# ai4ce/DiscoNet

Measured on AMD Instinct MI355X. Metric: scenes/sec (5-agent 256x256 BEV), higher is better.
Workload: dtype f16 hi+lo pair per value (32 bits; 22-bit significand for |x| >= 0.125, f16 exponent range, lo subnormal below: absolute floor 2^-25); conv products as split-f16 x3 MFMA, f32 accumulate; 1 GPU; DiscoNet det eval forward (--com disco), 5-agent, batch 4 per GPU, 256x256x13 BEV, no KD, sparse voxel lists -> dense -> enc -> DiscoGraph fusion -> dec -> cls/reg heads; agents=5, batch_per_gpu=4, conv_math=sp, launch=hipGraph replay, parallelism=scene-parallel x1 (no data-path collective)

## Files before the change

### disconet_amd/_lib.py

```python
import ctypes
import os
from ctypes import (POINTER, Structure, c_char_p, c_double, c_float, c_int, c_int32, c_long, c_longlong, c_size_t,
                    c_uint64, c_void_p)

_HERE = os.path.dirname(os.path.abspath(__file__))
LIB_PATH = os.environ.get("DISCONET_HIP_LIB") or os.path.join(_HERE, "libdisconet_hip.so")


class DnError(RuntimeError):
    pass


class ConvDesc(Structure):
    _fields_ = [(n, c_int32) for n in (
        "n_images", "h_in", "w_in", "c0", "c1", "up0", "c_out", "ksize", "stride", "relu",
        "ld0", "ld1", "ldo", "math")]


class PackJob(Structure):
    _fields_ = [("desc", ConvDesc), ("weight", c_void_p), ("packed", c_void_p), ("mode", c_int32), ("cin_total", c_int32),
                ("ci_first", c_int32), ("n_in", c_int32), ("wmul", c_float), ("reserved", c_int32)]


class FoldJob(Structure):
# ... 69 lines not shown
    "dn_conv_pack_multi_prepare": (c_int, [POINTER(PackJob), c_int, c_void_p, POINTER(c_int)]),
    "dn_conv_pack_weights_multi": (c_int, [c_void_p, c_int, c_int, c_void_p]),
    "dn_spconv2d": (c_int, [POINTER(ConvDesc), c_void_p, c_void_p, c_void_p, c_void_p, c_void_p,
                            c_void_p, c_void_p]),
    "dn_spconv_ks_supported": (c_int, [POINTER(ConvDesc), c_int]),
    "dn_spconv_workspace_bytes": (c_size_t, [POINTER(ConvDesc), c_int]),
    "dn_spconv2d_ks": (c_int, [POINTER(ConvDesc), c_int, c_void_p, c_void_p, c_void_p, c_void_p, c_void_p, c_void_p,
                               c_void_p, c_int, c_void_p, c_size_t, c_void_p]),
    "dn_spconv2d_pre_pair_supported": (c_int, [POINTER(ConvDesc), POINTER(ConvDesc)]),
    "dn_spconv2d_pre_pair": (c_int, [POINTER(ConvDesc), POINTER(ConvDesc), c_void_p, c_void_p, c_void_p, c_void_p, c_void_p,
                                     c_void_p, c_void_p, c_void_p, c_void_p]),
    "dn_spconv2d_dual": (c_int, [POINTER(ConvDesc), c_void_p, c_void_p, c_void_p, c_void_p, c_void_p,
                                 c_void_p, c_void_p, c_int, c_void_p]),
    "dn_spconv2d_nhwc": (c_int, [POINTER(ConvDesc), c_void_p, c_void_p, c_void_p, c_void_p, c_void_p, c_void_p, c_int,
                                 c_void_p]),
    "dn_sp_post1x1_packed_bytes": (c_size_t, []),
    "dn_sp_post1x1_pack_weights": (c_int, [c_void_p, c_int, c_int, c_float, c_void_p, c_void_p]),
    "dn_sp_post1x1_pack_heads": (c_int, [c_void_p, c_int, c_int, c_float, c_void_p, c_void_p]),
    "dn_spconv2d_post1x1": (c_int, [POINTER(ConvDesc), POINTER(Post1x1Desc)] + [c_void_p] * 8 +
                            [c_int, c_void_p, c_void_p, c_void_p]),
    "dn_spconv_force_config": (c_int, [c_int]),
    "dn_spconv_set_upmode": (c_int, [c_int]),
    "dn_spconv_last_form": (c_int, [POINTER(c_int), c_int]),
    "dn_conv_force_config": (c_int, [c_int]),
    "dn_conv_last_form": (c_int, [POINTER(c_int), c_int]),
    "dn_decode_boxes": (c_int, [c_void_p, c_void_p, c_void_p, c_int, c_long, c_void_p, c_void_p,
                                c_void_p]),
    "dn_detect_workspace_bytes": (c_size_t, [c_int, c_long, c_int]),
    "dn_detect": (c_int, [c_void_p, c_void_p, c_void_p, c_int, c_long, c_int, c_int, c_float, c_double, c_void_p,
                          c_void_p, c_void_p, c_void_p, c_void_p, c_size_t, c_void_p]),
    "dn_late_fuse_workspace_bytes": (c_size_t, [c_int, c_int, c_int, c_int, c_int, c_int]),
    "dn_late_fuse": (c_int, [c_void_p, c_void_p, c_void_p, c_void_p, c_void_p, c_int, c_int, c_int, c_int, c_int, c_int,
                             c_int, c_double, c_int, POINTER(c_double), c_void_p, c_void_p, c_void_p, c_void_p, c_void_p,
                             c_size_t, c_void_p]),
    "dn_ap_match_workspace_bytes": (c_size_t, [c_int, c_int, c_int, c_int]),
    "dn_ap_match": (c_int, [c_void_p, c_void_p, c_void_p, c_void_p, c_void_p, c_int, c_int, c_int, POINTER(c_double), c_int,
                            c_void_p, c_void_p, c_void_p, c_void_p, c_void_p, c_size_t, c_void_p, c_longlong, c_void_p, c_int,
                            c_int, c_void_p]),
    "dn_ap_reset": (c_int, [c_void_p, c_int, c_void_p]),
    "dn_gt_strata": (c_int, [c_void_p, c_void_p, c_void_p, c_int, c_int, c_int, POINTER(c_double), c_int, c_void_p, c_void_p]),
    "dn_ap_match_strata_workspace_bytes": (c_size_t, [c_int, c_int, c_int, c_int, c_int]),
    "dn_ap_match_strata": (c_int, [c_void_p, c_void_p, c_void_p, c_void_p, c_void_p, c_void_p, c_int, c_int, c_int,
                                   POINTER(c_double), c_int, c_int, c_void_p, c_void_p, c_void_p, c_void_p, c_void_p,
                                   c_void_p, c_size_t, c_void_p, c_longlong, c_void_p, c_int, c_int, c_void_p]),
    "dn_ap_strata_reset": (c_int, [c_void_p, c_int, c_int, c_void_p]),
    "dn_assign_targets_workspace_bytes": (c_size_t, [c_int, c_long, c_int]),
# ... 169 lines not shown
```

### disconet_amd/csrc/conv_sp.hip

```cpp
#ifndef DN_PHASE_TIMING
#define DN_PHASE_TIMING 0
#endif
#ifndef DN_SP_ABL
#define DN_SP_ABL 0
#endif
#include "dn_internal.h"
#include "sp_layout.h"
#include "sp_device.h"
#include "sp_split.h"
#include <array>
#include <cstdlib>
#include <type_traits>
#include <utility>

#if DN_PHASE_TIMING
__device__ unsigned long long g_phase_cycles[8];
extern "C" int dn_sp_phase_cycles(unsigned long long* host8, int reset) {
  if (hipDeviceSynchronize() != hipSuccess) return -1;
  if (host8 && hipMemcpyFromSymbol(host8, HIP_SYMBOL(g_phase_cycles), sizeof(unsigned long long) * 8) != hipSuccess) return -1;
  if (reset) { unsigned long long z[8] = {0}; if (hipMemcpyToSymbol(HIP_SYMBOL(g_phase_cycles), z, sizeof z) != hipSuccess) return -1; }
  return 0;
}
#endif

// ... 1146 lines not shown
             "spconv: a bit-grid source 0 (math = 4) needs a 3x3 stride-1 single-source layer of <= 32 channels");
  DN_REQUIRE(!d->up0 || (d->h_in % 2 == 0 && d->w_in % 2 == 0), "spconv: x2-upsampled source needs even h_in/w_in");
  DN_REQUIRE(d->c1 == 0 || (d->c0 % 16 == 0 && d->ksize == 3), "spconv: concat needs 3x3 and c0 %% 16 == 0 (c0 = %d)", d->c0);
  const size_t hs0 = d->up0 ? d->h_in / 2 : d->h_in, ws0 = d->up0 ? d->w_in / 2 : d->w_in;
  DN_REQUIRE(hs0 * ws0 * chunks_of(d->c0) * 64 < (1ull << 31) &&
                 (size_t)d->h_in * d->w_in * chunks_of(d->c1) * 64 < (1ull << 31),
             "spconv: one image must stay below 2 GiB");
  return DN_OK;
}

inline size_t packed_blocks(const dn_conv_desc& d) {
  const int nch = packed_chunks(d);
  if (up_mode(d) == 2) return dn::spq_packed_blocks(chunks_of(d.c0), nch);
  if (up_merged(d)) return (size_t)chunks_of(d.c0) * 12 + (size_t)(nch - chunks_of(d.c0)) * 9;
  return (size_t)nch * d.ksize * d.ksize;
}

enum SpCfgId { S3_256x64, S3_256x32, S3_128x64, S3_64x64, S3S2_128x64, S3S2_64x64, S1_256x64, S1_64x64,
               S3_256x64_T9, S3_512x64, S3_256x128, S1_256x64_C1, S3_256x32_ST, S3_64x64_T9, S3_128x64_T9,
               S3S2_64x64_T9, S3S2_128x64_T9, SP_CFG_COUNT };
enum SpForceId {
  FORCE_SPQ_BN32 = 20, FORCE_SPQ_BN64 = 21, FORCE_SPQ_DEEP = 22,
  FORCE_SPQ_ABL = 22,
  FORCE_TOOLS = 100,
  FORCE_ABL_256x64 = 100, FORCE_ABL_256x32 = 200,
  FORCE_ABL_64x64_T9 = 300,
  FORCE_ABL_S2_64x64 = 400,
};

template <int KS_, int STRIDE_, int TH_, int TW_, int BN_, int TG_, int CA_, int WAVES_M_, int WAVES_N_, int WTM_, int WTN_>
struct Geom {
  using G = Geom;
  static constexpr int KS = KS_, STRIDE = STRIDE_, TH = TH_, TW = TW_, BN = BN_, TG = TG_, CA = CA_, WAVES_M = WAVES_M_,
                       WAVES_N = WAVES_N_, WTM = WTM_, WTN = WTN_;
};
template <SpCfgId ID> struct Tile;
#define SP_TILE(id, bias_, deep_, ...) \
  template <> struct Tile<id> : __VA_ARGS__ { static constexpr float bias = bias_; static constexpr SpCfgId deep = deep_; }
SP_TILE(S3_256x64,      1.00f, S3_256x64_T9,   Geom<3, 1, 8,  32, 64,  3, 1, 4, 1, 2, 2>);
SP_TILE(S3_256x32,      1.15f, S3_256x32,      Geom<3, 1, 8,  32, 32,  3, 1, 4, 1, 2, 1>);
SP_TILE(S3_128x64,      1.10f, S3_128x64_T9,   Geom<3, 1, 8,  16, 64,  3, 1, 2, 2, 2, 1>);
SP_TILE(S3_64x64,       1.40f, S3_64x64_T9,    Geom<3, 1, 8,  8,  64,  3, 1, 2, 2, 1, 1>);
SP_TILE(S3S2_128x64,    1.45f, S3S2_128x64_T9, Geom<3, 2, 8,  16, 64,  3, 1, 2, 2, 2, 1>);
SP_TILE(S3S2_64x64,     1.00f, S3S2_64x64_T9,  Geom<3, 2, 8,  8,  64,  3, 1, 2, 2, 1, 1>);
SP_TILE(S1_256x64,      1.00f, S1_256x64,      Geom<1, 1, 8,  32, 64,  1, 2, 4, 1, 2, 2>);
SP_TILE(S1_64x64,       1.30f, S1_64x64,       Geom<1, 1, 8,  8,  64,  1, 4, 2, 2, 1, 1>);
// ... 356 lines not shown
}

extern "C" int dn_spconv_force_config(int cfg) {
  g_sp_force = cfg;
  return DN_OK;
}

extern "C" int dn_spconv_set_upmode(int mode) {
  g_sp_upmode = mode;
  return DN_OK;
}

namespace dn { SpLastForm g_sp_last_form = {-1, 0, 0, 0, 0, 0, 0, 0, 0, 0, 0, 0, 0, 0, 0, 0, 0, 0, 0, 0}; }

extern "C" int dn_spconv_last_form(int* out, int n) {
  constexpr int kInts = (int)(sizeof(dn::SpLastForm) / sizeof(int));
  static_assert(sizeof(dn::SpLastForm) == 20 * sizeof(int), "dn_spconv_last_form: the record is 20 ints");
  DN_REQUIRE(out && n > 0, "spconv last form: null pointer / no room");
  const int* f = reinterpret_cast<const int*>(&dn::g_sp_last_form);
  for (int i = 0; i < n && i < kInts; ++i) out[i] = f[i];
  return kInts;
}

namespace {
int spconv2d_impl(const dn_conv_desc* d, const void* src0, const void* src1, const void* packed, const float* scale,
                  const float* shift, void* out, float* out_nhwc, int ld_nhwc, void* stream, int kslices = 1,
                  void* workspace = nullptr, size_t workspace_bytes = 0);
}

extern "C" int dn_spconv2d(const dn_conv_desc* d, const void* src0, const void* src1,
                           const void* packed, const float* scale, const float* shift, void* out,
                           void* stream) {
  return spconv2d_impl(d, src0, src1, packed, scale, shift, out, nullptr, 0, stream);
}

extern "C" int dn_spconv2d_dual(const dn_conv_desc* d, const void* src0, const void* src1, const void* packed,
                                const float* scale, const float* shift, void* out_sp, float* out_nhwc, int ld_nhwc,
                                void* stream) {
  DN_REQUIRE(d && out_nhwc && ld_nhwc >= d->c_out && ld_nhwc % 4 == 0 && d->c_out % 4 == 0 &&
                 (reinterpret_cast<uintptr_t>(out_nhwc) & 15) == 0,
             "spconv dual: the fp32 NHWC output needs c_out %% 4 == 0, ld >= c_out, ld %% 4 == 0, 16-byte alignment");
  return spconv2d_impl(d, src0, src1, packed, scale, shift, out_sp, out_nhwc, ld_nhwc, stream);
}

extern "C" int dn_spconv2d_nhwc(const dn_conv_desc* d, const void* src0, const void* src1, const void* packed,
                                const float* scale, const float* shift, float* out_nhwc, int ld_nhwc, void* stream) {
// ... 26 lines not shown
  DN_REQUIRE(!out_nhwc || (d && ld_nhwc >= d->c_out && ld_nhwc % 4 == 0 && d->c_out % 4 == 0 &&
                           (reinterpret_cast<uintptr_t>(out_nhwc) & 15) == 0),
             "spconv: the fp32 NHWC output needs c_out %% 4 == 0, ld >= c_out, ld %% 4 == 0, 16-byte alignment");
  return spconv2d_impl(d, src0, src1, packed, scale, shift, out, out_nhwc, ld_nhwc, stream, kslices, workspace, workspace_bytes);
}

namespace {
int spconv2d_impl(const dn_conv_desc* d, const void* src0, const void* src1, const void* packed, const float* scale,
                  const float* shift, void* out, float* out_nhwc, int ld_nhwc, void* stream, int kslices,
                  void* workspace, size_t workspace_bytes) {
  if (int rc = validate(d)) return rc;
  DN_REQUIRE(src0 && packed && scale && shift && (out || out_nhwc), "spconv: null pointer");
  DN_REQUIRE(d->c1 == 0 || src1, "spconv: c1 > 0 but src1 is null");
  SpArgs a;
  if (int rc = fill_args(d, src0, src1, packed, scale, shift, out, a)) return rc;
  a.out_b = out_nhwc; a.ldo_b = ld_nhwc;
  DN_REQUIRE(!out_nhwc || g_sp_force < FORCE_TOOLS, "spconv dual: not with a forced tools configuration");
  hipStream_t s = (hipStream_t)stream;
  DN_REQUIRE(kslices == 1 || (ks_layer(*d) && a.c0g + a.c1g >= kslices),
             "spconv: %d K slices need a 3x3 layer of at least that many 16-channel chunks", kslices);
  if (up_mode(*d) == 2) {
    DN_REQUIRE(a.c1g == 0 || d->c0 % 16 == 0, "spconv: concat needs c0 %% 16 == 0");
    const int f = g_sp_force;
    const int bn = f == FORCE_SPQ_BN32 ? 32 : f == FORCE_SPQ_BN64 ? 64 : f == FORCE_SPQ_DEEP ? 33 :
                   (f > FORCE_SPQ_ABL && f <= FORCE_SPQ_ABL + 3) ? 100 + (f - FORCE_SPQ_ABL) : 0;
    return dn::spq_conv(d, src0, src1, packed, (size_t)a.wpk_bytes, scale, shift, out, a.cout_pad, bn, s, kslices,
                        (float*)workspace, workspace_bytes, out_nhwc, ld_nhwc);
  }
  if (kslices > 1) {
    a.ks.count = kslices;
    a.ks.partial = (float*)workspace;
    a.ks_ws_bytes = workspace_bytes;
    const SpCfg c = select_cfg(*d, kslices, workspace != nullptr && workspace_bytes > 0);
    const int rc = launch_form<KSliced, S3_256x32, S3_128x64, S3_64x64, S3S2_128x64, S3S2_64x64, S3_64x64_T9, S3_128x64_T9,
                               S3S2_64x64_T9, S3S2_128x64_T9>(c.id, a, *d, s);
    return rc != kNotListed ? rc : dn::fail(DN_ERR_UNSUPPORTED, "spconv: tile configuration %d has no K-sliced form", (int)c.id);
  }
  if (d->math == 3) {
    if (fits_stationary<HiOnlyStationary, S3_256x32>(*d, 0, 2)) return launch_form<HiOnlyStationary, S3_256x32>(a, *d, s);
    return launch_form<HiOnly, S3_256x32>(a, *d, s);
  }
  if (d->math == 4) {
    if (fits_stationary<BitGrid, S3_256x32>(*d, 0, 2)) return launch_form<BitGrid, S3_256x32>(a, *d, s);
    return dn::fail(DN_ERR_UNSUPPORTED, "spconv: a bit-grid source needs a layer whose weights fit the LDS (c_out <= 32)");
  }
  const SpCfg c = select_cfg(*d);
  if (up_merged(*d)) {
// ... 74 lines not shown
```

### disconet_amd/csrc/conv_spq.hip

```cpp
#ifndef DN_SP_ABL
#define DN_SP_ABL 0
#endif
#include "dn_internal.h"
#include "sp_layout.h"
#include "sp_device.h"
#include "sp_split.h"
#include <type_traits>

namespace {

constexpr int kCUs = 256;

constexpr int QTH = 8, QTW = 32, QPH = QTH + 2, QPW = QTW + 2, QHALF = QPW / 2, QPITCH = QPW, QNPIX = QPH * QPITCH;
constexpr int QNW = 4, QNT = QNW * 64;
constexpr int QA_PIECES = 4 * QNPIX;
constexpr int QA_INSTR = (QA_PIECES + 63) / 64;
constexpr int QA_IT = (QA_INSTR + QNW - 1) / QNW;
constexpr int QA_STAGE = QA_INSTR * 1024;
static_assert(QA_INSTR == 22 && QA_IT == 6, "patch stage: 22 instructions, waves 0 / 1 issue 6, waves 2 / 3 issue 5");

struct SpqArgs {
  const unsigned char* src0;
  const unsigned char* src1;
  const unsigned char* wpk;
// ... 15 lines not shown
struct QTile {
  int img, oy0, ox0, n0;
};

template <int BN, int DEEP = 0>
struct SpqTile {
  static constexpr int WTN = BN / 32;
  static constexpr int TGQ = DEEP ? 4 : (BN == 64 ? 1 : 2);
  static constexpr int NS0 = 4 / TGQ;
  static constexpr int TG1 = DEEP ? 9 : 3;
  static constexpr int NS1 = 9 / TG1;
  static constexpr int BLK = 4 * BN * 16;
  static constexpr int B_PIECES0 = TGQ * 4 * 4 * BN;
  static constexpr int B_PIECES1 = TG1 * 4 * BN;
  static constexpr int B_IT0 = (B_PIECES0 + QNT - 1) / QNT;
  static constexpr int B_IT1 = (B_PIECES1 + QNT - 1) / QNT;
  static_assert(B_IT1 <= B_IT0, "the source-0 step is the larger one");
  static constexpr int QB_STAGE = B_IT0 * QNT * 16;
  static constexpr int AFF_BYTES = QNW * 2 * 64 * 4;
  static constexpr int LDS_BYTES = 2 * QA_STAGE + 2 * QB_STAGE + AFF_BYTES;
  static_assert((DEEP ? 1 : 2) * LDS_BYTES <= 160 * 1024, "two workgroups per CU (DEEP: one)");
};

template <int BN, int DEEP, int ABL = 0, int KSL = 0>
__global__ void __launch_bounds__(QNT, 2) conv_spq_kernel(const SpqArgs a) {
  static_assert(!KSL || BN == 32, "K slices: the 32-channel tile");
  using T = SpqTile<BN, DEEP>;
  constexpr int WTN = T::WTN, TGQ = T::TGQ, NS0 = T::NS0, NS1 = T::NS1, BLK = T::BLK, QB_STAGE = T::QB_STAGE;
  extern __shared__ __attribute__((aligned(16))) unsigned char smem[];
  constexpr int OFF_B = 2 * QA_STAGE;

  const int tid = threadIdx.x;
  const int lane = tid & 63;
  const int wave = tid >> 6;
  const int li = lane & 31, lh = lane >> 5;
  const int py = wave & 1, px = wave >> 1;

  const int G = gridDim.x;
  const int spatial_items = a.n_images * a.tiles_y * a.tiles_x;
  const int n_cb = a.n_cb;
  const int sp_full = spatial_items & ~7;
  auto decode = [&](int item) {
    QTile tc;
    int cb, spi;
    if (item < sp_full * n_cb) {
      const int j = item >> 3;
      const int jq = fdivmod(j, n_cb, a.rcp_ncb, cb);
      spi = (item & 7) * (sp_full >> 3) + jq;
    } else {
// ... 98 lines not shown
  };
  int voffb_n0 = -1;
  auto setup_voff_b = [&](const QTile& tc) {
    if (tc.n0 == voffb_n0) return;
    voffb_n0 = tc.n0;
    const int t = opaque(tid);
#pragma unroll
    for (int it = 0; it < T::B_IT0; ++it) {
      const int piece = (it * QNW + (t >> 6)) * 64 + (t & 63);
      const int blk = piece / (4 * BN), q = (piece / BN) % 4, nn = piece % BN;
      voff_b[it] = (unsigned)(((blk * 4 + q) * a.cout_pad + tc.n0 + nn) * 16);
    }
  };
  auto setup_rsrc = [&](const QTile& tc) {
    rsrc0 = __builtin_amdgcn_make_buffer_rsrc(const_cast<unsigned char*>(a.src0 + tc.img * img0_bytes), 0,
                                              (int)img0_bytes, 0x00020000);
    rsrc1 = __builtin_amdgcn_make_buffer_rsrc(const_cast<unsigned char*>(a.c1g ? a.src1 + tc.img * img1_bytes : a.src0),
                                              0, a.c1g ? (int)img1_bytes : 0, 0x00020000);
  };
  auto issue_a = [&](int g, int sa) {
    if constexpr ((ABL & 2) != 0) return;
    const bool from1 = g >= a.c0g;
    const int soff = from1 ? (g - a.c0g) * 4 * (int)plane1 : g * 4 * (int)plane0;
    unsigned char* base = smem + sa * QA_STAGE + wave * 1024;
#pragma unroll
    for (int it = 0; it < QA_IT; ++it) {
      if (it == QA_IT - 1 && wave >= QA_INSTR - (QA_IT - 1) * QNW) break;
      if (from1)
        dma16(rsrc1, base + it * QNW * 1024, voff_a[it], soff);
      else
        dma16(rsrc0, base + it * QNW * 1024, voff_a[it], soff);
    }
  };
  auto issue_b = [&](int g, int st, int sb) {
    if constexpr ((ABL & 1) != 0) return;
    const bool from1 = g >= a.c0g;
    const int blk = from1 ? a.c0g * 16 + (g - a.c0g) * 9 + st * T::TG1 : g * 16 + st * (TGQ * 4);
    const int soff = blk * 4 * a.cout_pad * 16;
    unsigned char* base = smem + OFF_B + sb * QB_STAGE + wave * 1024;
#pragma unroll
    for (int it = 0; it < T::B_IT0; ++it)
      if (!from1 || it < T::B_IT1) dma16(rsrcw, base + it * QNW * 1024, voff_b[it], soff);
  };

  struct Frags {
    half8 ah[2], al[2], bh[WTN], bl[WTN];
  };
  auto mma = [&](const Frags& f) {
#pragma unroll
    for (int wm = 0; wm < 2; ++wm)
// ... 72 lines not shown
      __builtin_amdgcn_sched_barrier(0);
      load(std::integral_constant<int, 2>{});
      __builtin_amdgcn_sched_barrier(0);
      mma(f[1]);
      __builtin_amdgcn_sched_barrier(0);
      load(std::integral_constant<int, 3>{});
      __builtin_amdgcn_sched_barrier(0);
      mma(f[0]);
      __builtin_amdgcn_sched_barrier(0);
      mma(f[1]);
    } else if constexpr (TGQ == 2) {
      load(std::integral_constant<int, 1>{});
      __builtin_amdgcn_sched_barrier(0);
      mma(f[0]);
      __builtin_amdgcn_sched_barrier(0);
      mma(f[1]);
    } else {
      __builtin_amdgcn_sched_barrier(0);
      mma(f[0]);
    }
    __builtin_amdgcn_sched_barrier(0);
  };

  float* aff_s = reinterpret_cast<float*>(smem + 2 * QA_STAGE + 2 * QB_STAGE) + wave * 128;
  int aff_n0 = -1;
  auto load_affine = [&](int n0) {
    if (n0 == aff_n0) return;
    aff_n0 = n0;
    if (lane < BN) {
      const int co = n0 + lane, ci = min(co, a.c_out - 1);
      aff_s[lane] = co < a.c_out ? a.scale[ci] : 0.f;
      aff_s[64 + lane] = co < a.c_out ? a.shift[ci] : 0.f;
    }
  };
  auto epilogue = [&](const QTile& tc) {
    const int plane = a.h * a.w * 16;
    const int img_bytes = a.cog * 4 * plane;
    const auto rsrc_o = __builtin_amdgcn_make_buffer_rsrc(a.out + (size_t)tc.img * img_bytes, 0, img_bytes, 0x00020000);
    const float lo_clamp = a.relu ? 0.f : -65504.f;
    if (a.out_f32 != nullptr) {
      const float floor_v = a.relu ? 0.f : -__builtin_inff();
#pragma unroll
      for (int wm = 0; wm < 2; ++wm) {
        const int oy = tc.oy0 + prow[wm], ox = tc.ox0 + pcol;
        const bool inside = oy < a.h && ox < a.w;
        float* orow = a.out_f32 + (((size_t)tc.img * a.h + oy) * a.w + ox) * a.ldo_f32;
#pragma unroll
        for (int wn = 0; wn < WTN; ++wn)
#pragma unroll
          for (int g = 0; g < 4; ++g) {
            const int co = tc.n0 + 32 * wn + 8 * g + 4 * lh;
            const f32x4 sc = *reinterpret_cast<const f32x4*>(aff_s + wn * 32 + 8 * g + 4 * lh);
            const f32x4 sh = *reinterpret_cast<const f32x4*>(aff_s + 64 + wn * 32 + 8 * g + 4 * lh);
            f32x4 v = affine4(quad_of(acc[wm][wn], g), sc, sh);
            nan_seen |= !(fabsf(v[0]) <= 3.4028235e38f) | !(fabsf(v[1]) <= 3.4028235e38f) | !(fabsf(v[2]) <= 3.4028235e38f) |
                        !(fabsf(v[3]) <= 3.4028235e38f);
#pragma unroll
            for (int e = 0; e < 4; ++e) v[e] = fmaxf(v[e], floor_v);
            if (inside && co < a.c_out) *reinterpret_cast<f32x4*>(orow + co) = v;
          }
      }
      if (a.out == nullptr) return;
    }
#pragma unroll
    for (int wm = 0; wm < 2; ++wm) {
      const int oy = tc.oy0 + prow[wm], ox = tc.ox0 + pcol;
      const bool inside = oy < a.h && ox < a.w;
      const int voff = inside ? (oy * a.w + ox) * 16 + lh * plane : (int)0x80000000;
#pragma unroll
      for (int wn = 0; wn < WTN; ++wn) {
        u32x2 hi[4], lo[4];
#pragma unroll
        for (int g = 0; g < 4; ++g) {
          const f32x4 sc = *reinterpret_cast<const f32x4*>(aff_s + wn * 32 + 8 * g + 4 * lh);
          const f32x4 sh = *reinterpret_cast<const f32x4*>(aff_s + 64 + wn * 32 + 8 * g + 4 * lh);
          const f32x4 v = affine4(quad_of(acc[wm][wn], g), sc, sh);
          split4(v, hi[g], lo[g], amax, lo_clamp);
        }
#pragma unroll
        for (int m = 0; m < 2; ++m) {
          const u32x4 ph = gather_octet(hi[2 * m], hi[2 * m + 1]);
          const u32x4 pl = gather_octet(lo[2 * m], lo[2 * m + 1]);
          const int cg = (tc.n0 + 32 * wn) / 16 + m;
          if (cg < a.cog) {
            __builtin_amdgcn_raw_buffer_store_b128(ph, rsrc_o, voff + cg * 4 * plane, 0, 0);
            __builtin_amdgcn_raw_buffer_store_b128(pl, rsrc_o, voff + (cg * 4 + 2) * plane, 0, 0);
          }
        }
      }
    }
  };

  int item = blockIdx.x;
  if (item >= a.total_items) return;
  auto partial_of = [&](int j) {
    return a.ks.partial + ((size_t)j * QNW + wave) * (2 * WTN * 16 * 64) + lane * 4;
  };
  auto fold_acc = [&]() {
// ... 33 lines not shown
        const QTile tc = decode(a.ks.n_whole + p);
        load_affine(tc.n0);
        zero_tot();
        for (int sl = 0; sl < a.ks.count; ++sl) {
          const float* pb = partial_of((p << a.ks.log2) + sl);
#pragma unroll
          for (int wm = 0; wm < 2; ++wm)
#pragma unroll
            for (int wn = 0; wn < WTN; ++wn)
#pragma unroll
              for (int q = 0; q < 4; ++q) {
                const f32x4 v = *reinterpret_cast<const f32x4*>(pb + ((wm * WTN + wn) * 4 + q) * 256);
#pragma unroll
                for (int e = 0; e < 4; ++e) acc[wm][wn][4 * q + e] = v[e];
              }
          fold_acc();
        }
        tot_to_acc();
        epilogue(tc);
        note_range(amax, nan_seen);
      }
      return;
    }
  }
  Work cw = decode_work(item);
  QTile cur = cw.tc;
  setup_rsrc(cur);
  setup_voff_b(cur);
  setup_voff_a(cur, first_group(cw) >= a.c0g);
  issue_b(first_group(cw), 0, 0);
  issue_a(first_group(cw), 0);
  int sa = 0, sb = 0;
  bool a_pending = true;

  while (true) {
#pragma unroll
    for (int wm = 0; wm < 2; ++wm)
#pragma unroll
      for (int wn = 0; wn < WTN; ++wn)
#pragma unroll
        for (int r = 0; r < 16; ++r) acc[wm][wn][r] = 0.f;
    load_affine(cur.n0);
    const bool has_next = item + G < a.total_items;
    QTile nxt = cur;
    int ng0 = 0;
    if (has_next) {
// ... 108 lines not shown
      dx0 = b == 0 ? 0 : (px == 0 ? 1 : 2);  dx1 = b == 0 ? (px == 0 ? 0 : 1) : 2;
    } else {
      const long q = r - (long)c0g * 16;
      cg = c0g + (int)(q / 9);
      dy0 = dy1 = (int)(q % 9) / 3;
      dx0 = dx1 = (int)(q % 3);
    }
    float v[8];
#pragma unroll
    for (int e = 0; e < 8; ++e) {
      const int ci = cg * 16 + oct * 8 + e;
      v[e] = 0.f;
      if (n < c_out && ci < c_in) {
        const float* wp = w + ((size_t)n * c_in + ci) * 9;
        for (int dy = dy0; dy <= dy1; ++dy)
          for (int dx = dx0; dx <= dx1; ++dx) v[e] += wp[dy * 3 + dx];
        v[e] *= wmul;
      }
    }
    sp::split_store(wpk, sp::weight_piece(r, sp::quarter_of(0, oct), cout_pad, n), (size_t)2 * cout_pad, v);
  }
}

template <int BN, int DEEP = 0, int ABL = 0, int KSL = 0>
int launch_spq(SpqArgs& a, hipStream_t stream, size_t ws_bytes = 0) {
  using T = SpqTile<BN, DEEP>;
  auto kern = conv_spq_kernel<BN, DEEP, ABL, KSL>;
  static dn::PerDeviceFlag attr_flag;
  bool& attr_set = attr_flag.here();
  if (!attr_set) {
    hipError_t e = hipFuncSetAttribute(reinterpret_cast<const void*>(kern), hipFuncAttributeMaxDynamicSharedMemorySize,
                                       (int)T::LDS_BYTES);
    if (e != hipSuccess)
      return dn::fail(DN_ERR_LAUNCH, "spconv (quad-merged): hipFuncSetAttribute(%d B LDS): %s", (int)T::LDS_BYTES,
                      hipGetErrorString(e));
    attr_set = true;
  }
  a.tiles_x = (a.w + QTW - 1) / QTW;
  a.tiles_y = (a.h + QTH - 1) / QTH;
  const long total = (long)a.n_images * a.tiles_y * a.tiles_x * ((a.c_out + BN - 1) / BN);
  DN_REQUIRE(total < (1L << 22), "spconv (quad-merged): too many tiles (%ld)", total);
  DN_REQUIRE((long)a.h * a.w * 16 * 4 * a.cog < (1L << 31), "spconv (quad-merged): one output image exceeds 2 GiB");
  a.total_items = (int)total;
  a.n_cb = (a.c_out + BN - 1) / BN;
  a.rcp_ncb = 1.0f / (float)a.n_cb; a.rcp_tx = 1.0f / (float)a.tiles_x; a.rcp_ty = 1.0f / (float)a.tiles_y;
  const long resident = (DEEP ? 1L : 2L) * kCUs;
  dn::SpLastForm form = {1, 3, 1, QTH, QTW, BN, 0, 1, 0, 0, 2, 0, KSL, 0, DEEP, 0, 0, 0, 0, 0};
  if constexpr (KSL != 0) {
    KSlices& k = a.ks;
    const int S = k.count, ng = a.c0g + a.c1g;
    DN_REQUIRE((S == 2 || S == 4) && ng >= S, "spconv (quad-merged): %d K slices of a %d-chunk layer", S, ng);
    const long wtot = 4L * a.c0g + 9L * a.c1g;
    int b[5] = {0, 0, 0, 0, ng};
    for (int sl = 1; sl < S; ++sl) {
      int g = b[sl - 1] + 1;
      auto before = [&](int gg) { return gg <= a.c0g ? 4L * gg : 4L * a.c0g + 9L * (gg - a.c0g); };
      while (g < ng - (S - 1 - sl) - 1 && before(g) * S < wtot * sl) ++g;
      b[sl] = g;
    }
    k.log2 = S == 4 ? 2 : 1; k.ngroups = ng;
    k.b1 = b[1]; k.b2 = S == 2 ? ng : b[2]; k.b3 = S == 2 ? ng : b[3];
    const size_t per_tile = (size_t)S * QNW * 2 * (BN / 32) * 16 * 64 * sizeof(float);
    k.n_whole = (int)ks_plan(total, resident, S, k.partial ? ws_bytes : 0, per_tile);
    k.n_split = (int)(total - k.n_whole);
    k.fixup = 0;
    const long work = k.n_whole + (long)k.n_split * S;
    a.total_items = (int)work;
    form.grid = (int)(work > resident ? resident : work); form.total_items = (int)work;
    form.n_whole = k.n_whole; form.n_split = k.n_split;
    form.fixup_grid = k.n_split ? (int)(k.n_split > 2 * kCUs ? 2 * kCUs : k.n_split) : 0;
    dn::g_sp_last_form = form;
    hipLaunchKernelGGL(kern, dim3((unsigned)(work > resident ? resident : work)), dim3(QNT), T::LDS_BYTES, stream, a);
    if (k.n_split) {
      k.fixup = 1;
      a.total_items = k.n_split;
      hipLaunchKernelGGL(kern, dim3((unsigned)(k.n_split > 2 * kCUs ? 2 * kCUs : k.n_split)), dim3(QNT), T::LDS_BYTES, stream, a);
    }
    return dn::check_launch("conv_spq_kernel (K slices)");
  }
  dim3 grid((unsigned)(total > resident ? resident : total));
  form.grid = (int)grid.x; form.total_items = (int)total; form.n_whole = (int)total;
  dn::g_sp_last_form = form;
  hipLaunchKernelGGL(kern, grid, dim3(QNT), T::LDS_BYTES, stream, a);
  return dn::check_launch("conv_spq_kernel");
}

}

namespace dn {

void range_collect_conv_spq(unsigned* dst, bool reset, hipStream_t s) { sp_range_collect_here(dst, reset, s); }

size_t spq_packed_blocks(int c0g, int nchunks) { return (size_t)c0g * 16 + (size_t)(nchunks - c0g) * 9; }

int spq_pack_weights(const float* weight_oihw, void* packed, int c_out, int c_in, int c0g, int cout_pad, int nchunks,
                     float wmul, hipStream_t stream) {
  hipLaunchKernelGGL(spq_pack_weights_kernel, dim3(2048), dim3(256), 0, stream, weight_oihw, (unsigned char*)packed, c_out,
                     c_in, c0g, cout_pad, nchunks, wmul);
  return check_launch("spq_pack_weights_kernel");
}

int spq_conv(const dn_conv_desc* d, const void* src0, const void* src1, const void* packed, size_t packed_bytes,
             const float* scale, const float* shift, void* out, int cout_pad, int bn, hipStream_t stream,
             int kslices, float* workspace, size_t workspace_bytes, float* out_nhwc, int ld_nhwc) {
  SpqArgs a;
  a.src0 = (const unsigned char*)src0; a.src1 = (const unsigned char*)src1; a.wpk = (const unsigned char*)packed;
  a.scale = scale; a.shift = shift; a.out = (unsigned char*)out;
  a.out_f32 = out_nhwc; a.ldo_f32 = ld_nhwc;
  a.n_images = d->n_images; a.h = d->h_in; a.w = d->w_in;
  a.c0g = (d->c0 + 15) / 16; a.c1g = (d->c1 + 15) / 16;
  a.c_out = d->c_out; a.cog = (d->c_out + 15) / 16; a.relu = d->relu;
  a.cout_pad = cout_pad; a.wpk_bytes = (int)packed_bytes;
  a.tiles_x = a.tiles_y = a.total_items = 0;
  a.ks = KSlices{workspace, kslices, 0, 0, 0, 0, 0, 0, 0, 0};
  if (kslices > 1) {
    const long tiles = (long)d->n_images * ((d->h_in + QTH - 1) / QTH) * ((d->w_in + QTW - 1) / QTW);
    const bool deep = tiles * ((d->c_out + 31) / 32) * kslices <= (long)kCUs;
    if (bn == 33 || (bn == 0 && deep)) return launch_spq<32, 1, 0, 1>(a, stream, workspace_bytes);
    return launch_spq<32, 0, 0, 1>(a, stream, workspace_bytes);
  }
  if (bn == 0) {
    const long tiles = (long)d->n_images * ((d->h_in + QTH - 1) / QTH) * ((d->w_in + QTW - 1) / QTW);
    bn = (d->c_out > 32 && tiles * ((d->c_out + 63) / 64) >= 4L * kCUs) ? 64 : 32;
    if (bn == 32 && tiles * ((d->c_out + 31) / 32) <= (long)kCUs) bn = 33;
  }
  if (bn == 64) return launch_spq<64>(a, stream);
  if (bn == 33) return launch_spq<32, 1>(a, stream);
#if DN_SP_ABL
  if (bn == 101) return launch_spq<32, 0, 1>(a, stream);
  if (bn == 102) return launch_spq<32, 0, 2>(a, stream);
  if (bn == 103) return launch_spq<32, 0, 3>(a, stream);
#endif
  return launch_spq<32>(a, stream);
}

}
```

### disconet_amd/csrc/dn_internal.h

```cpp
#pragma once
#include <hip/hip_runtime.h>
#include <cstdarg>
#include <cstdio>

#include "disconet_hip.h"

namespace dn {

char* err_buf();

inline int fail(int code, const char* fmt, ...) {
  va_list ap;
  va_start(ap, fmt);
  vsnprintf(err_buf(), 512, fmt, ap);
  va_end(ap);
  return code;
}

hipError_t zero_fill(void* ptr, size_t bytes, hipStream_t stream);

struct PerDeviceFlag {
  bool done[64] = {};
  bool& here() {
    int dev = 0;
// ... 30 lines not shown
int spq_conv(const dn_conv_desc* d, const void* src0, const void* src1, const void* packed, size_t packed_bytes,
             const float* scale, const float* shift, void* out, int cout_pad, int bn, hipStream_t stream,
             int kslices = 1, float* workspace = nullptr, size_t workspace_bytes = 0, float* out_nhwc = nullptr,
             int ld_nhwc = 0);

int fuse_mlp_agent_scores(const float* feat, const float* warped, int warped_fm, const int32_t* num_agent,
                          const dn_fuse_mlp_params* p, const float* w5, int batch, int agents, int hw, int c, int only_v2i,
                          int ego_first, int ego_count, float* partials, hipStream_t stream);

void range_collect_conv_sp(unsigned* dst, bool reset, hipStream_t stream);
void range_collect_conv_spq(unsigned* dst, bool reset, hipStream_t stream);
void range_collect_fuse_mlp(unsigned* dst, bool reset, hipStream_t stream);
void range_collect_conv_wgrad(unsigned* dst, bool reset, hipStream_t stream);
unsigned* sp_range_word();

struct SpLastForm {
  int family;
  int ks, stride, th, tw, bn, tg, ca, post, bstat, upm, ahi, ksl, nb, deep;
  int grid, total_items;
  int n_whole, n_split;
  int fixup_grid;
};
extern SpLastForm g_sp_last_form;

}

#define DN_REQUIRE(cond, ...) \
  do { if (!(cond)) return dn::fail(DN_ERR_ARG, __VA_ARGS__); } while (0)

#define DN_REQUIRE_EVAL_STEP(who, max_m, max_g)                                                                \
  DN_REQUIRE(rect, who ": null rect");                                                                         \
  DN_REQUIRE(id, who ": null id");                                                                             \
  DN_REQUIRE(count, who ": null count");                                                                       \
  DN_REQUIRE(gt_boxes, who ": null gt_boxes");                                                                 \
  DN_REQUIRE(gt_ids, who ": null gt_ids");                                                                     \
  DN_REQUIRE(gt_count, who ": null gt_count");                                                                 \
  DN_REQUIRE(state, who ": null state");                                                                       \
  DN_REQUIRE(m >= 1 && m <= (max_m), who ": M = %d track rows, must be in [1, %d]", m, (max_m));              \
  DN_REQUIRE(g >= 1 && g <= (max_g), who ": G = %d ground-truth rows, must be in [1, %d]", g, (max_g));       \
  DN_REQUIRE(std::isfinite(scale) && scale > 0, who ": scale = %g, must be finite and > 0", scale)
```

### disconet_amd/ops.py

```python
import ctypes
import os

import torch

from . import _lib
from ._lib import ConvDesc, FuseMlpParams, MlpTailParams, Post1x1Desc, check


def _ptr(t):
    return ctypes.c_void_p(t.data_ptr()) if t is not None else None


def _stream_handle():
    return torch._C._cuda_getCurrentRawStream(torch._C._cuda_getDevice())


def _stream():
    return ctypes.c_void_p(_stream_handle())


def _need_gpu(*tensors):
    for t in tensors:
        if t is not None and not t.is_cuda:
            raise _lib.DnError("disconet_amd ops need tensors on the MI355X (got a %s tensor); "
# ... 490 lines not shown
    if (tuple(out.shape) != (d.n_images, ho, wo, d.c_out) or out.dtype != torch.float32 or out.stride(3) != 1
            or out.stride(1) != wo * out.stride(2) or out.stride(0) != ho * out.stride(1)):
        raise _lib.DnError("sp_conv2d_nhwc: out must be float32 [n, h_out, w_out, c_out] rows (a channel slice is fine)")
    if src0.hi_only or src0.bits or (src1 is not None and (src1.hi_only or src1.bits)):
        raise _lib.DnError("sp_conv2d_nhwc: full SP sources only")
    check(_lib.load().dn_spconv2d_nhwc(ctypes.byref(d), _ptr(src0.data), _ptr(src1.data) if src1 is not None else None,
                                       _ptr(packed), _ptr(scale), _ptr(shift), _ptr(out), out.stride(2), _stream()),
          "dn_spconv2d_nhwc")
    return out


SP_FORM_FIELDS = ("family", "KS", "STRIDE", "TH", "TW", "BN", "TG", "CA", "POST", "BSTAT", "UPM", "AHI", "KSL", "NB", "DEEP",
                  "grid", "total_items", "n_whole", "n_split", "fixup_grid")


def sp_last_form():
    buf = (ctypes.c_int * len(SP_FORM_FIELDS))()
    n = _lib.load().dn_spconv_last_form(buf, len(SP_FORM_FIELDS))
    if n != len(SP_FORM_FIELDS):
        raise _lib.DnError("dn_spconv_last_form: %d fields, expected %d" % (n, len(SP_FORM_FIELDS)))
    return dict(zip(SP_FORM_FIELDS, (int(v) for v in buf)))


def sp_conv2d_pre_pair_supported(d1, d2):
    return bool(_lib.load().dn_spconv2d_pre_pair_supported(ctypes.byref(d1), ctypes.byref(d2)))


def sp_conv2d_pre_pair(d1, d2, bits, packed1, scale1, shift1, packed2, scale2, shift2, out=None):
    _need_gpu(bits, packed1, packed2, scale1, shift1, scale2, shift2)
    if not getattr(bits, "bits", False):
        raise _lib.DnError("sp_conv2d_pre_pair: the source must be an occupancy bit grid (ops.scatter_dense_bits)")
    if out is None:
        out = SpTensor(d2.n_images, d2.h_in, d2.w_in, d2.c_out, device=bits.device)
    check(_lib.load().dn_spconv2d_pre_pair(ctypes.byref(d1), ctypes.byref(d2), _ptr(bits.data), _ptr(packed1), _ptr(scale1),
                                           _ptr(shift1), _ptr(packed2), _ptr(scale2), _ptr(shift2), _ptr(out.data), _stream()),
          "dn_spconv2d_pre_pair")
    return out


def sp_pack_post1x1_weights(weight):
    _need_gpu(weight)
    w = weight.detach().reshape(weight.shape[0], -1).contiguous().float()
    lib = _lib.load()
    wmul = _pow2_lift(w)
    packed = torch.empty(lib.dn_sp_post1x1_packed_bytes(), dtype=torch.uint8, device=weight.device)
    check(lib.dn_sp_post1x1_pack_weights(_ptr(w), w.shape[0], w.shape[1], wmul, _ptr(packed), _stream()),
# ... 316 lines not shown
```

### include/disconet_hip.h

```cpp
#ifndef DISCONET_HIP_H
#define DISCONET_HIP_H

#include <stddef.h>
#include <stdint.h>

#ifdef __cplusplus
extern "C" {
#endif

#define DN_OK 0
#define DN_ERR_ARG (-1)
#define DN_ERR_LAUNCH (-2)
#define DN_ERR_UNSUPPORTED (-3)

int dn_version(void);
const char* dn_build_id(void);
const char* dn_last_error(void);

unsigned dn_sp_range_flags(int reset);
int dn_sp_range_flags_async(unsigned* dst_device, int reset, void* stream);

int dn_voxelize_occupy(const float* pts, int n_pts, int pt_stride,
                       const double* voxel_size_host, const double* extents_host,
                       const int* dims_host, float* dense, void* stream);
// ... 89 lines not shown

int dn_spconv2d_pre_pair_supported(const dn_conv_desc* d1, const dn_conv_desc* d2);
int dn_spconv2d_pre_pair(const dn_conv_desc* d1, const dn_conv_desc* d2, const uint32_t* bits, const void* packed1,
                         const float* scale1, const float* shift1, const void* packed2, const float* scale2,
                         const float* shift2, void* out_sp, void* stream);
int dn_spconv2d_dual(const dn_conv_desc* d, const void* src0_sp, const void* src1_sp, const void* packed,
                     const float* scale, const float* shift, void* out_sp, float* out_nhwc, int ld_nhwc,
                     void* stream);
int dn_spconv2d_nhwc(const dn_conv_desc* d, const void* src0_sp, const void* src1_sp, const void* packed,
                     const float* scale, const float* shift, float* out_nhwc, int ld_nhwc, void* stream);
size_t dn_sp_post1x1_packed_bytes(void);
int dn_sp_post1x1_pack_weights(const float* w2, int c_out2, int c_in2, float wmul, void* packed,
                               void* stream);
int dn_sp_post1x1_pack_heads(const float* w2, int c_out2, int split, float wmul, void* packed,
                             void* stream);
int dn_spconv2d_post1x1(const dn_conv_desc* d, const dn_post1x1_desc* p, const void* src0_sp,
                        const void* src1_sp, const void* packed, const float* scale,
                        const float* shift, const void* packed2, const float* scale2,
                        const float* shift2, int out_f32, void* out_a, float* out_b, void* stream);
int dn_spconv_force_config(int cfg);
int dn_spconv_set_upmode(int mode);
int dn_spconv_last_form(int* out, int n);

int dn_conv_force_config(int cfg);
int dn_conv_last_form(int* out, int n);

int dn_warp_neighbors(const float* feat, const float* trans, const int32_t* num_agent,
                      int batch, int agents, int h, int w, int c, int only_v2i,
                      int ego_first, int ego_count, float* warped, void* stream);

#define DN_FUSE_SUM 0
#define DN_FUSE_MEAN 1
#define DN_FUSE_MAX 2
int dn_fuse_reduce(const float* feat, const float* trans, const int32_t* num_agent, int batch, int agents, int h, int w,
                   int c, int only_v2i, int ego_first, int ego_count, int mode, float* fused, void* stream);

typedef struct dn_mlp_tail_params {
  const float* bn1_scale; const float* bn1_shift;
  const float* w2; const float* s2; const float* t2;
  const float* w3; const float* s3; const float* t3;
  const float* w4; const float* b4;
} dn_mlp_tail_params;

int dn_disco_fuse_tail(const float* feat, const float* warped, const float* g,
                       const float* fw, const int32_t* num_agent,
                       const dn_mlp_tail_params* p, int batch, int agents, int hw, int c,
// ... 165 lines not shown
```

Measured before the change: 2431 scenes/s.

## Keep quad-merged conv weights resident in registers and LDS for small layers

Adds a resident-weights variant of the quad-merged 32-channel spconv kernel. For layers with at most 4+2 input chunks, c_out <= 32 and no K slices, it loads the first source's weights once into registers and the second source's 3x3 weight blocks into LDS. Only activation tiles are then streamed per work item. This removes the repeated per-tile weight staging (B-stage DMA) and shrinks the LDS footprint, at the cost of higher register pressure from holding 32 half8 weight fragments per lane. It also adds a query entry point that reports whether the last launch used this path.

```diff
diff --git a/disconet_amd/_lib.py b/disconet_amd/_lib.py
--- a/disconet_amd/_lib.py
+++ b/disconet_amd/_lib.py
@@ -115,6 +115,7 @@
     "dn_spconv_force_config": (c_int, [c_int]),
     "dn_spconv_set_upmode": (c_int, [c_int]),
     "dn_spconv_last_form": (c_int, [POINTER(c_int), c_int]),
+    "dn_spconv_last_resident": (c_int, []),
     "dn_conv_force_config": (c_int, [c_int]),
     "dn_conv_last_form": (c_int, [POINTER(c_int), c_int]),
     "dn_decode_boxes": (c_int, [c_void_p, c_void_p, c_void_p, c_int, c_long, c_void_p, c_void_p,
diff --git a/disconet_amd/csrc/conv_sp.hip b/disconet_amd/csrc/conv_sp.hip
--- a/disconet_amd/csrc/conv_sp.hip
+++ b/disconet_amd/csrc/conv_sp.hip
@@ -1192,6 +1192,7 @@
 enum SpForceId {
   FORCE_SPQ_BN32 = 20, FORCE_SPQ_BN64 = 21, FORCE_SPQ_DEEP = 22,
   FORCE_SPQ_ABL = 22,
+  FORCE_SPQ_RES = 26,
   FORCE_TOOLS = 100,
   FORCE_ABL_256x64 = 100, FORCE_ABL_256x32 = 200,
   FORCE_ABL_64x64_T9 = 300,
@@ -1594,6 +1595,10 @@
   return kInts;
 }
 
+extern "C" int dn_spconv_last_resident(void) {
+  return dn::g_sp_last_form.family == 1 && dn::g_spq_last_resident ? 1 : 0;
+}
+
 namespace {
 int spconv2d_impl(const dn_conv_desc* d, const void* src0, const void* src1, const void* packed, const float* scale,
                   const float* shift, void* out, float* out_nhwc, int ld_nhwc, void* stream, int kslices = 1,
@@ -1666,7 +1671,7 @@
   if (up_mode(*d) == 2) {
     DN_REQUIRE(a.c1g == 0 || d->c0 % 16 == 0, "spconv: concat needs c0 %% 16 == 0");
     const int f = g_sp_force;
-    const int bn = f == FORCE_SPQ_BN32 ? 32 : f == FORCE_SPQ_BN64 ? 64 : f == FORCE_SPQ_DEEP ? 33 :
+    const int bn = f == FORCE_SPQ_BN32 ? 32 : f == FORCE_SPQ_BN64 ? 64 : f == FORCE_SPQ_DEEP ? 33 : f == FORCE_SPQ_RES ? 34 :
                    (f > FORCE_SPQ_ABL && f <= FORCE_SPQ_ABL + 3) ? 100 + (f - FORCE_SPQ_ABL) : 0;
     return dn::spq_conv(d, src0, src1, packed, (size_t)a.wpk_bytes, scale, shift, out, a.cout_pad, bn, s, kslices,
                         (float*)workspace, workspace_bytes, out_nhwc, ld_nhwc);
diff --git a/disconet_amd/csrc/conv_spq.hip b/disconet_amd/csrc/conv_spq.hip
--- a/disconet_amd/csrc/conv_spq.hip
+++ b/disconet_amd/csrc/conv_spq.hip
@@ -1,5 +1,8 @@
 #ifndef DN_SP_ABL
 #define DN_SP_ABL 0
+#endif
+#ifndef DN_SPQ_RES
+#define DN_SPQ_RES 1
 #endif
 #include "dn_internal.h"
 #include "sp_layout.h"
@@ -61,9 +64,23 @@
   static_assert((DEEP ? 1 : 2) * LDS_BYTES <= 160 * 1024, "two workgroups per CU (DEEP: one)");
 };
 
-template <int BN, int DEEP, int ABL = 0, int KSL = 0>
+struct SpqRes {
+  static constexpr int C0G = 4, C1G = 2;
+  static constexpr int A_STAGE = QA_PIECES * 16;
+  static constexpr int BLK = 4 * 32 * 16;
+  static constexpr int W1_INSTR = C1G * 9 * BLK / 1024;
+  static constexpr int OFF_W1 = 2 * A_STAGE;
+  static constexpr int OFF_AFF = OFF_W1 + C1G * 9 * BLK;
+  static constexpr int LDS_BYTES = OFF_AFF + 2 * 32 * 4;
+  static_assert(W1_INSTR % QNW == 0, "the second source's blocks: whole rounds of DMA instructions");
+  static_assert(2 * LDS_BYTES <= 160 * 1024, "two workgroups per CU");
+};
+
+template <int BN, int DEEP, int ABL = 0, int KSL = 0, int RES = 0>
 __global__ void __launch_bounds__(QNT, 2) conv_spq_kernel(const SpqArgs a) {
   static_assert(!KSL || BN == 32, "K slices: the 32-channel tile");
+  static_assert(!RES || (BN == 32 && !DEEP && !KSL && !ABL), "resident weights: the plain 32-channel tile");
+  constexpr int A_STRIDE = RES ? SpqRes::A_STAGE : QA_STAGE;
   using T = SpqTile<BN, DEEP>;
   constexpr int WTN = T::WTN, TGQ = T::TGQ, NS0 = T::NS0, NS1 = T::NS1, BLK = T::BLK, QB_STAGE = T::QB_STAGE;
   extern __shared__ __attribute__((aligned(16))) unsigned char smem[];
@@ -208,10 +225,13 @@
     if constexpr ((ABL & 2) != 0) return;
     const bool from1 = g >= a.c0g;
     const int soff = from1 ? (g - a.c0g) * 4 * (int)plane1 : g * 4 * (int)plane0;
-    unsigned char* base = smem + sa * QA_STAGE + wave * 1024;
+    unsigned char* base = smem + sa * A_STRIDE + wave * 1024;
 #pragma unroll
     for (int it = 0; it < QA_IT; ++it) {
       if (it == QA_IT - 1 && wave >= QA_INSTR - (QA_IT - 1) * QNW) break;
+      if constexpr (RES != 0) {
+        if (it == QA_IT - 1 && (it * QNW + wave) * 64 + lane >= QA_PIECES) break;
+      }
       if (from1)
         dma16(rsrc1, base + it * QNW * 1024, voff_a[it], soff);
       else
@@ -330,7 +350,9 @@
     __builtin_amdgcn_sched_barrier(0);
   };
 
-  float* aff_s = reinterpret_cast<float*>(smem + 2 * QA_STAGE + 2 * QB_STAGE) + wave * 128;
+  constexpr int AFF_SH = RES ? 32 : 64;
+  float* aff_s = RES ? reinterpret_cast<float*>(smem + SpqRes::OFF_AFF)
+                     : reinterpret_cast<float*>(smem + 2 * QA_STAGE + 2 * QB_STAGE) + wave * 128;
   int aff_n0 = -1;
   auto load_affine = [&](int n0) {
     if (n0 == aff_n0) return;
@@ -338,8 +360,13 @@
     if (lane < BN) {
       const int co = n0 + lane, ci = min(co, a.c_out - 1);
       aff_s[lane] = co < a.c_out ? a.scale[ci] : 0.f;
-      aff_s[64 + lane] = co < a.c_out ? a.shift[ci] : 0.f;
-    }
+      aff_s[AFF_SH + lane] = co < a.c_out ? a.shift[ci] : 0.f;
+    }
+  };
+  auto aff_of_tile = [&]() {
+    int ao = 0;
+    if constexpr (RES != 0) asm volatile("" : "+v"(ao));
+    return aff_s + ao;
   };
   auto epilogue = [&](const QTile& tc) {
     const int plane = a.h * a.w * 16;
@@ -353,13 +380,14 @@
         const int oy = tc.oy0 + prow[wm], ox = tc.ox0 + pcol;
         const bool inside = oy < a.h && ox < a.w;
         float* orow = a.out_f32 + (((size_t)tc.img * a.h + oy) * a.w + ox) * a.ldo_f32;
+        const float* aff = aff_of_tile();
 #pragma unroll
         for (int wn = 0; wn < WTN; ++wn)
 #pragma unroll
           for (int g = 0; g < 4; ++g) {
             const int co = tc.n0 + 32 * wn + 8 * g + 4 * lh;
-            const f32x4 sc = *reinterpret_cast<const f32x4*>(aff_s + wn * 32 + 8 * g + 4 * lh);
-            const f32x4 sh = *reinterpret_cast<const f32x4*>(aff_s + 64 + wn * 32 + 8 * g + 4 * lh);
+            const f32x4 sc = *reinterpret_cast<const f32x4*>(aff + wn * 32 + 8 * g + 4 * lh);
+            const f32x4 sh = *reinterpret_cast<const f32x4*>(aff + AFF_SH + wn * 32 + 8 * g + 4 * lh);
             f32x4 v = affine4(quad_of(acc[wm][wn], g), sc, sh);
             nan_seen |= !(fabsf(v[0]) <= 3.4028235e38f) | !(fabsf(v[1]) <= 3.4028235e38f) | !(fabsf(v[2]) <= 3.4028235e38f) |
                         !(fabsf(v[3]) <= 3.4028235e38f);
@@ -375,13 +403,14 @@
       const int oy = tc.oy0 + prow[wm], ox = tc.ox0 + pcol;
       const bool inside = oy < a.h && ox < a.w;
       const int voff = inside ? (oy * a.w + ox) * 16 + lh * plane : (int)0x80000000;
+      const float* aff = aff_of_tile();
 #pragma unroll
       for (int wn = 0; wn < WTN; ++wn) {
         u32x2 hi[4], lo[4];
 #pragma unroll
         for (int g = 0; g < 4; ++g) {
-          const f32x4 sc = *reinterpret_cast<const f32x4*>(aff_s + wn * 32 + 8 * g + 4 * lh);
-          const f32x4 sh = *reinterpret_cast<const f32x4*>(aff_s + 64 + wn * 32 + 8 * g + 4 * lh);
+          const f32x4 sc = *reinterpret_cast<const f32x4*>(aff + wn * 32 + 8 * g + 4 * lh);
+          const f32x4 sh = *reinterpret_cast<const f32x4*>(aff + AFF_SH + wn * 32 + 8 * g + 4 * lh);
           const f32x4 v = affine4(quad_of(acc[wm][wn], g), sc, sh);
           split4(v, hi[g], lo[g], amax, lo_clamp);
         }
@@ -461,6 +490,137 @@
       }
       return;
     }
+  }
+  if constexpr (RES != 0) {
+    using R = SpqRes;
+    const int w1_instr = a.c1g * (9 * R::BLK / 1024);
+#pragma unroll
+    for (int it = 0; it < R::W1_INSTR / QNW; ++it) {
+      const int ins = it * QNW + wave;
+      const int piece = ins * 64 + lane;
+      const unsigned vo = (unsigned)((((piece >> 7) * 4 + ((piece >> 5) & 3)) * a.cout_pad + (piece & 31)) * 16);
+      if (ins < w1_instr) dma16(rsrcw, smem + R::OFF_W1 + ins * 1024, vo, a.c0g * 16 * 4 * a.cout_pad * 16);
+    }
+    half8 wh[R::C0G][4], wl[R::C0G][4];
+#pragma unroll
+    for (int g = 0; g < R::C0G; ++g)
+#pragma unroll
+      for (int t = 0; t < 4; ++t) {
+        const unsigned vo = (unsigned)((((g * 16 + t * 4 + wave) * 4 + lh) * a.cout_pad + li) * 16);
+        const unsigned vh = g < a.c0g ? vo : OOB, vl = g < a.c0g ? vo + (unsigned)(2 * a.cout_pad * 16) : OOB;
+        wh[g][t] = __builtin_bit_cast(half8, __builtin_amdgcn_raw_buffer_load_b128(rsrcw, vh, 0, 0));
+        wl[g][t] = __builtin_bit_cast(half8, __builtin_amdgcn_raw_buffer_load_b128(rsrcw, vl, 0, 0));
+      }
+    load_affine(0);
+    __builtin_amdgcn_s_waitcnt(0x0F70);
+    __builtin_amdgcn_s_barrier();
+    asm volatile("" ::: "memory");
+
+    QTile cur = decode(item);
+    setup_rsrc(cur);
+    setup_voff_a(cur, false);
+    issue_a(0, 0);
+    int sa = 0;
+    auto compute0r = [&](const unsigned char* As, const half8 (&bh)[4], const half8 (&bl)[4]) {
+      Frags f[2];
+      auto load = [&](auto t_c) {
+        constexpr int t = decltype(t_c)::value, am = t >> 1, b = t & 1;
+        Frags& d = f[t & 1];
+#pragma unroll
+        for (int wm = 0; wm < 2; ++wm) {
+          d.ah[wm] = *reinterpret_cast<const half8*>(As + a_b0[wm][b][am]);
+          d.al[wm] = *reinterpret_cast<const half8*>(As + a_b0[wm][b][am] + 2 * QNPIX * 16);
+        }
+        d.bh[0] = bh[t];
+        d.bl[0] = bl[t];
+      };
+      load(std::integral_constant<int, 0>{});
+      load(std::integral_constant<int, 1>{});
+      __builtin_amdgcn_sched_barrier(0);
+      mma(f[0]);
+      __builtin_amdgcn_sched_barrier(0);
+      load(std::integral_constant<int, 2>{});
+      __builtin_amdgcn_sched_barrier(0);
+      mma(f[1]);
+      __builtin_amdgcn_sched_barrier(0);
+      load(std::integral_constant<int, 3>{});
+      __builtin_amdgcn_sched_barrier(0);
+      mma(f[0]);
+      __builtin_amdgcn_sched_barrier(0);
+      mma(f[1]);
+      __builtin_amdgcn_sched_barrier(0);
+    };
+    auto compute1r = [&](const unsigned char* As, const unsigned char* Bs) {
+      Frags f[2];
+      auto load_a = [&](int u) {
+        Frags& d = f[u & 1];
+#pragma unroll
+        for (int wm = 0; wm < 2; ++wm) {
+          d.ah[wm] = *reinterpret_cast<const half8*>(As + a_b1[wm][u % 3] + (u / 3) * QPITCH * 16);
+          d.al[wm] = *reinterpret_cast<const half8*>(As + a_b1[wm][u % 3] + (u / 3) * QPITCH * 16 + 2 * QNPIX * 16);
+        }
+      };
+      half8 bh, bl;
+      auto load_b = [&](int u) {
+        bh = *reinterpret_cast<const half8*>(Bs + b_off[0] + u * BLK);
+        bl = *reinterpret_cast<const half8*>(Bs + b_off[0] + u * BLK + 2 * BN * 16);
+      };
+      load_a(0);
+      load_b(0);
+#pragma unroll
+      for (int u = 0; u < 9; ++u) {
+        if (u + 1 < 9) load_a(u + 1);
+        __builtin_amdgcn_sched_barrier(0);
+        f[u & 1].bh[0] = bh;
+        f[u & 1].bl[0] = bl;
+        mma(f[u & 1]);
+        __builtin_amdgcn_sched_barrier(0);
+        if (u + 1 < 9) load_b(u + 1);
+      }
+      __builtin_amdgcn_sched_barrier(0);
+    };
+    while (true) {
+#pragma unroll
+      for (int wm = 0; wm < 2; ++wm)
+#pragma unroll
+        for (int r = 0; r < 16; ++r) acc[wm][0][r] = 0.f;
+      const bool has_next = item + G < a.total_items;
+      QTile nxt = cur;
+      if (has_next) nxt = decode(item + G);
+      auto hand_over = [&](int g) {
+        wait_vm0();
+        __builtin_amdgcn_s_barrier();
+        asm volatile("" ::: "memory");
+        if (g + 1 < nchunks) {
+          if (g + 1 == a.c0g) setup_voff_a(cur, true);
+          issue_a(g + 1, sa ^ 1);
+        } else if (has_next) {
+          setup_rsrc(nxt);
+          setup_voff_a(nxt, false);
+          issue_a(0, sa ^ 1);
+        }
+      };
+#pragma unroll
+      for (int g = 0; g < R::C0G; ++g)
+        if (g < a.c0g) {
+          hand_over(g);
+          compute0r(smem + sa * A_STRIDE, wh[g], wl[g]);
+          sa ^= 1;
+        }
+      for (int g1 = 0; g1 < a.c1g; ++g1) {
+        hand_over(a.c0g + g1);
+        const unsigned char* As = smem + sa * A_STRIDE;
+        const unsigned char* Bs = smem + R::OFF_W1 + g1 * 9 * R::BLK;
+        compute1r(As, Bs);
+        sa ^= 1;
+      }
+      epilogue(cur);
+      note_range(amax, nan_seen);
+      if (!has_next) break;
+      item += G;
+      cur = nxt;
+    }
+    return;
   }
   Work cw = decode_work(item);
   QTile cur = cw.tc;
@@ -615,17 +775,18 @@
   }
 }
 
-template <int BN, int DEEP = 0, int ABL = 0, int KSL = 0>
+template <int BN, int DEEP = 0, int ABL = 0, int KSL = 0, int RES = 0>
 int launch_spq(SpqArgs& a, hipStream_t stream, size_t ws_bytes = 0) {
   using T = SpqTile<BN, DEEP>;
-  auto kern = conv_spq_kernel<BN, DEEP, ABL, KSL>;
+  auto kern = conv_spq_kernel<BN, DEEP, ABL, KSL, RES>;
+  constexpr int LDS_BYTES = RES ? (int)SpqRes::LDS_BYTES : (int)T::LDS_BYTES;
   static dn::PerDeviceFlag attr_flag;
   bool& attr_set = attr_flag.here();
   if (!attr_set) {
     hipError_t e = hipFuncSetAttribute(reinterpret_cast<const void*>(kern), hipFuncAttributeMaxDynamicSharedMemorySize,
-                                       (int)T::LDS_BYTES);
+                                       LDS_BYTES);
     if (e != hipSuccess)
-      return dn::fail(DN_ERR_LAUNCH, "spconv (quad-merged): hipFuncSetAttribute(%d B LDS): %s", (int)T::LDS_BYTES,
+      return dn::fail(DN_ERR_LAUNCH, "spconv (quad-merged): hipFuncSetAttribute(%d B LDS): %s", LDS_BYTES,
                       hipGetErrorString(e));
     attr_set = true;
   }
@@ -639,6 +800,7 @@
   a.rcp_ncb = 1.0f / (float)a.n_cb; a.rcp_tx = 1.0f / (float)a.tiles_x; a.rcp_ty = 1.0f / (float)a.tiles_y;
   const long resident = (DEEP ? 1L : 2L) * kCUs;
   dn::SpLastForm form = {1, 3, 1, QTH, QTW, BN, 0, 1, 0, 0, 2, 0, KSL, 0, DEEP, 0, 0, 0, 0, 0};
+  dn::g_spq_last_resident = RES;
   if constexpr (KSL != 0) {
     KSlices& k = a.ks;
     const int S = k.count, ng = a.c0g + a.c1g;
@@ -674,7 +836,7 @@
   dim3 grid((unsigned)(total > resident ? resident : total));
   form.grid = (int)grid.x; form.total_items = (int)total; form.n_whole = (int)total;
   dn::g_sp_last_form = form;
-  hipLaunchKernelGGL(kern, grid, dim3(QNT), T::LDS_BYTES, stream, a);
+  hipLaunchKernelGGL(kern, grid, dim3(QNT), LDS_BYTES, stream, a);
   return dn::check_launch("conv_spq_kernel");
 }
 
@@ -692,6 +854,8 @@
                      c_in, c0g, cout_pad, nchunks, wmul);
   return check_launch("spq_pack_weights_kernel");
 }
+
+int g_spq_last_resident = 0;
 
 int spq_conv(const dn_conv_desc* d, const void* src0, const void* src1, const void* packed, size_t packed_bytes,
              const float* scale, const float* shift, void* out, int cout_pad, int bn, hipStream_t stream,
@@ -706,6 +870,7 @@
   a.cout_pad = cout_pad; a.wpk_bytes = (int)packed_bytes;
   a.tiles_x = a.tiles_y = a.total_items = 0;
   a.ks = KSlices{workspace, kslices, 0, 0, 0, 0, 0, 0, 0, 0};
+  const bool resident_ok = a.c0g <= SpqRes::C0G && a.c1g <= SpqRes::C1G && d->c_out <= 32 && kslices <= 1;
   if (kslices > 1) {
     const long tiles = (long)d->n_images * ((d->h_in + QTH - 1) / QTH) * ((d->w_in + QTW - 1) / QTW);
     const bool deep = tiles * ((d->c_out + 31) / 32) * kslices <= (long)kCUs;
@@ -716,6 +881,12 @@
     const long tiles = (long)d->n_images * ((d->h_in + QTH - 1) / QTH) * ((d->w_in + QTW - 1) / QTW);
     bn = (d->c_out > 32 && tiles * ((d->c_out + 63) / 64) >= 4L * kCUs) ? 64 : 32;
     if (bn == 32 && tiles * ((d->c_out + 31) / 32) <= (long)kCUs) bn = 33;
+    if (DN_SPQ_RES && bn == 32 && resident_ok) bn = 34;
+  }
+  if (bn == 34) {
+    DN_REQUIRE(resident_ok, "spconv (quad-merged): the resident-weights form takes <= %d + %d chunks, c_out <= 32, no K slices",
+               SpqRes::C0G, SpqRes::C1G);
+    return launch_spq<32, 0, 0, 0, 1>(a, stream);
   }
   if (bn == 64) return launch_spq<64>(a, stream);
   if (bn == 33) return launch_spq<32, 1>(a, stream);
diff --git a/disconet_amd/csrc/dn_internal.h b/disconet_amd/csrc/dn_internal.h
--- a/disconet_amd/csrc/dn_internal.h
+++ b/disconet_amd/csrc/dn_internal.h
@@ -76,6 +76,7 @@
   int fixup_grid;
 };
 extern SpLastForm g_sp_last_form;
+extern int g_spq_last_resident;
 
 }
 
diff --git a/disconet_amd/ops.py b/disconet_amd/ops.py
--- a/disconet_amd/ops.py
+++ b/disconet_amd/ops.py
@@ -536,6 +536,10 @@
     return dict(zip(SP_FORM_FIELDS, (int(v) for v in buf)))
 
 
+def sp_last_resident():
+    return bool(_lib.load().dn_spconv_last_resident())
+
+
 def sp_conv2d_pre_pair_supported(d1, d2):
     return bool(_lib.load().dn_spconv2d_pre_pair_supported(ctypes.byref(d1), ctypes.byref(d2)))
 
diff --git a/include/disconet_hip.h b/include/disconet_hip.h
--- a/include/disconet_hip.h
+++ b/include/disconet_hip.h
@@ -135,6 +135,8 @@
 int dn_spconv_set_upmode(int mode);
 int dn_spconv_last_form(int* out, int n);
 
+int dn_spconv_last_resident(void);
+
 int dn_conv_force_config(int cfg);
 int dn_conv_last_form(int* out, int n);
 
```

Measured after the change: 2473 scenes/s, median of 6. 1.8% higher.
